# apple/ml-cvnets

Hardware: NVIDIA H100
Metric: images/sec training step, MobileViTv2-1.0 bf16 256x256 (higher is better)
Workload: dtype bf16

## Files before the change

### ml-cvnets_b200/csrc/common.cuh

```cuda
#pragma once
#include <cuda_bf16.h>
#include <cuda_runtime.h>
#include <stdint.h>
#include <stdio.h>
#include <string.h>

#include "../../include/cvnets_b200.h"

#if defined(__CUDA_ARCH__) && (__CUDA_ARCH__ != 900)
#error "libcvnets_b200 targets sm_90a (H100) only"
#endif

typedef __nv_bfloat16 bf16;
typedef __nv_bfloat162 bf162;

void cvb_set_error(const char* fmt, ...);
#define CVB_CHECK(cond, ...)            \
  do {                                  \
    if (!(cond)) {                      \
      cvb_set_error(__VA_ARGS__);       \
      return 1;                         \
    }                                   \
  } while (0)
#define CVB_CUDA(call)                                                                   \
  do {                                                                                   \
    cudaError_t e_ = (call);                                                             \
    if (e_ != cudaSuccess) {                                                             \
      (void)cudaGetLastError();  \
      cvb_set_error("%s:%d CUDA error: %s", __FILE__, __LINE__, cudaGetErrorString(e_)); \
      return 2;                                                                          \
    }                                                                                    \
  } while (0)
#define CVB_LAUNCH_CHECK() CVB_CUDA(cudaGetLastError())

static inline bool cvb_aligned16(const void* p) { return (reinterpret_cast<uintptr_t>(p) & 15) == 0; }
int cvb_num_sms();
int cvb_det_alloc(double** scratch, size_t n, cudaStream_t st);
int cvb_det_add(const double* scratch, float* dst, int rows, int cols, int ld, cudaStream_t st);
int cvb_det_free(double* scratch, cudaStream_t st);

#ifndef CVB_SILU_EXP
#define CVB_SILU_EXP 0
#endif
__device__ __forceinline__ float tanh_approx_f(float x) {
  float y;
  asm("tanh.approx.f32 %0, %1;" : "=f"(y) : "f"(x));
  return y;
}
__device__ __forceinline__ float sigmoid_f(float z) {
#if CVB_SILU_EXP
  return 1.0f / (1.0f + __expf(-z));
#else
  return fmaf(0.5f, tanh_approx_f(0.5f * z), 0.5f);
#endif
}
__device__ __forceinline__ float silu_f(float z) {
#if CVB_SILU_EXP
  return z / (1.0f + __expf(-z));
#else
  const float h = 0.5f * z;
  return fmaf(h, tanh_approx_f(h), h);
#endif
}
__device__ __forceinline__ float silu_grad_f(float z) {
  const float s = sigmoid_f(z);
  return s * (1.0f + z * (1.0f - s));
}
__device__ __forceinline__ float bf16_round(float x) { return __bfloat162float(__float2bfloat16_rn(x)); }

__device__ __forceinline__ uint32_t pack_bf162(float lo, float hi) {
  bf162 v = __floats2bfloat162_rn(lo, hi);
  return *reinterpret_cast<uint32_t*>(&v);
}
__device__ __forceinline__ float2 unpack_bf162(uint32_t u) {
  bf162 v = *reinterpret_cast<bf162*>(&u);
  return __bfloat1622float2(v);
}
__device__ __forceinline__ float2 ffma2(float2 a, float2 b, float2 c) { return make_float2(__fmaf_rn(a.x, b.x, c.x), __fmaf_rn(a.y, b.y, c.y)); }
__device__ __forceinline__ float2 fmul2(float2 a, float2 b) { return make_float2(__fmul_rn(a.x, b.x), __fmul_rn(a.y, b.y)); }
__device__ __forceinline__ float2 fadd2(float2 a, float2 b) { return make_float2(__fadd_rn(a.x, b.x), __fadd_rn(a.y, b.y)); }
__device__ __forceinline__ void unpack8(const uint4& u, float* f) {
  float2 a = unpack_bf162(u.x), b = unpack_bf162(u.y), c = unpack_bf162(u.z), d = unpack_bf162(u.w);
  f[0] = a.x; f[1] = a.y; f[2] = b.x; f[3] = b.y; f[4] = c.x; f[5] = c.y; f[6] = d.x; f[7] = d.y;
}
__device__ __forceinline__ uint4 pack8(const float* f) {
  uint4 u;
  u.x = pack_bf162(f[0], f[1]); u.y = pack_bf162(f[2], f[3]); u.z = pack_bf162(f[4], f[5]); u.w = pack_bf162(f[6], f[7]);
  return u;
}
__device__ __forceinline__ uint4 ldg16(const void* p) { return __ldg(reinterpret_cast<const uint4*>(p)); }
__device__ __forceinline__ uint4 ldg16_stream(const void* p) {
  uint4 r;
  asm volatile("ld.global.nc.L1::no_allocate.v4.u32 {%0,%1,%2,%3}, [%4];" : "=r"(r.x), "=r"(r.y), "=r"(r.z), "=r"(r.w) : "l"(p));
  return r;
}
__device__ __forceinline__ void stg16(void* p, const uint4& v) { *reinterpret_cast<uint4*>(p) = v; }

__device__ __forceinline__ uint32_t smem_u32(const void* p) { return static_cast<uint32_t>(__cvta_generic_to_shared(p)); }

__device__ __forceinline__ void cp_async16(uint32_t smem_addr, const void* gptr, bool pred) {
  int sz = pred ? 16 : 0;
  asm volatile("cp.async.cg.shared.global [%0], [%1], 16, %2;\n" ::"r"(smem_addr), "l"(gptr), "r"(sz));
}
__device__ __forceinline__ void cp_async_commit() { asm volatile("cp.async.commit_group;\n" ::); }
template <int N>
__device__ __forceinline__ void cp_async_wait() { asm volatile("cp.async.wait_group %0;\n" ::"n"(N)); }

__device__ __forceinline__ void ldmatrix_x4(uint32_t addr, uint32_t& r0, uint32_t& r1, uint32_t& r2, uint32_t& r3) {
  asm volatile("ldmatrix.sync.aligned.m8n8.x4.shared.b16 {%0,%1,%2,%3}, [%4];\n" : "=r"(r0), "=r"(r1), "=r"(r2), "=r"(r3) : "r"(addr));
}
__device__ __forceinline__ void ldmatrix_x4_trans(uint32_t addr, uint32_t& r0, uint32_t& r1, uint32_t& r2, uint32_t& r3) {
  asm volatile("ldmatrix.sync.aligned.m8n8.x4.trans.shared.b16 {%0,%1,%2,%3}, [%4];\n" : "=r"(r0), "=r"(r1), "=r"(r2), "=r"(r3) : "r"(addr));
}
__device__ __forceinline__ void mma_bf16_16816(float* d, const uint32_t* a, uint32_t b0, uint32_t b1) {
  asm volatile(
      "mma.sync.aligned.m16n8k16.row.col.f32.bf16.bf16.f32 {%0,%1,%2,%3}, {%4,%5,%6,%7}, {%8,%9}, {%0,%1,%2,%3};\n"
      : "+f"(d[0]), "+f"(d[1]), "+f"(d[2]), "+f"(d[3])
      : "r"(a[0]), "r"(a[1]), "r"(a[2]), "r"(a[3]), "r"(b0), "r"(b1));
}

__device__ __forceinline__ float warp_sum(float v) {
#pragma unroll
  for (int o = 16; o > 0; o >>= 1) v += __shfl_xor_sync(0xffffffffu, v, o);
  return v;
}
__device__ __forceinline__ float warp_max(float v) {
#pragma unroll
  for (int o = 16; o > 0; o >>= 1) v = fmaxf(v, __shfl_xor_sync(0xffffffffu, v, o));
  return v;
}

__device__ __forceinline__ float apply_mode(int mode, float x, float p0, float p1) {
  switch (mode) {
    case CVB_A_AFF: return fmaf(p0, x, p1);
    case CVB_A_AFF_SILU: return silu_f(fmaf(p0, x, p1));
    case CVB_A_SILU: return silu_f(x);
    default: return x;
  }
}

__device__ __forceinline__ void pdl_wait() { asm volatile("griddepcontrol.wait;" ::: "memory"); }
__device__ __forceinline__ void pdl_trigger() { asm volatile("griddepcontrol.launch_dependents;" ::: "memory"); }
int cvb_pdl_enabled();
template <typename... KArgs, typename... Args>
static inline cudaError_t cvb_launch(void (*kernel)(KArgs...), dim3 grid, dim3 block, size_t smem, cudaStream_t st, Args&&... args) {
  cudaLaunchConfig_t cfg;
  memset(&cfg, 0, sizeof(cfg));
  cfg.gridDim = grid;
  cfg.blockDim = block;
  cfg.dynamicSmemBytes = smem;
  cfg.stream = st;
  cudaLaunchAttribute attr[1];
  attr[0].id = cudaLaunchAttributeProgrammaticStreamSerialization;
  attr[0].val.programmaticStreamSerializationAllowed = 1;
  cfg.attrs = attr;
  cfg.numAttrs = cvb_pdl_enabled() ? 1 : 0;
  return cudaLaunchKernelEx(&cfg, kernel, static_cast<KArgs>(args)...);
}

#include <cuda.h>

int cvb_make_tmap_nhwc(CUtensorMap* map, const void* base, int B, int H, int W, int C, int boxH, int boxW, int boxC, int swizzle128);
int cvb_make_tmap_2d_k32(CUtensorMap* map, const void* base, int64_t rows, int cols, int ld, int box_rows);
int cvb_make_tmap_2d_c64(CUtensorMap* map, const void* base, int64_t rows, int cols, int ld, int box_rows);

__device__ __forceinline__ void mbar_init(uint64_t* bar, uint32_t count) {
  asm volatile("mbarrier.init.shared::cta.b64 [%0], %1;" ::"r"(smem_u32(bar)), "r"(count) : "memory");
}
__device__ __forceinline__ void fence_mbar_init() { asm volatile("fence.mbarrier_init.release.cluster;" ::: "memory"); }
__device__ __forceinline__ void fence_proxy_async() { asm volatile("fence.proxy.async.shared::cta;" ::: "memory"); }
__device__ __forceinline__ void mbar_expect_tx(uint64_t* bar, uint32_t bytes) {
  asm volatile("mbarrier.arrive.expect_tx.shared::cta.b64 _, [%0], %1;" ::"r"(smem_u32(bar)), "r"(bytes) : "memory");
}
__device__ __forceinline__ void mbar_wait(uint64_t* bar, uint32_t parity) {
  asm volatile(
      "{\n\t"
      ".reg .pred P1;\n\t"
      "WAIT_LOOP:\n\t"
      "mbarrier.try_wait.parity.shared::cta.b64 P1, [%0], %1;\n\t"
      "@P1 bra WAIT_DONE;\n\t"
      "bra WAIT_LOOP;\n\t"
      "WAIT_DONE:\n\t"
      "}" ::"r"(smem_u32(bar)), "r"(parity)
      : "memory");
}
__device__ __forceinline__ void tma_load_2d(void* smem_dst, const CUtensorMap* map, uint64_t* bar, int col, int row) {
  asm volatile("cp.async.bulk.tensor.2d.shared::cluster.global.mbarrier::complete_tx::bytes [%0], [%1, {%3, %4}], [%2];" ::"r"(smem_u32(smem_dst)),
               "l"(reinterpret_cast<uint64_t>(map)), "r"(smem_u32(bar)), "r"(col), "r"(row)
               : "memory");
}
__device__ __forceinline__ void mbar_arrive(uint64_t* bar) { asm volatile("mbarrier.arrive.shared::cta.b64 _, [%0];" ::"r"(smem_u32(bar)) : "memory"); }

enum { WG_SW128 = 1, WG_SW64 = 2 };
__device__ __forceinline__ uint64_t wgmma_desc(uint32_t saddr, uint32_t lbo_bytes, uint32_t sbo_bytes, int layout) {
  uint64_t d = 0;
  d |= (uint64_t)((saddr & 0x3FFFFu) >> 4);
  d |= (uint64_t)((lbo_bytes >> 4) & 0x3FFFu) << 16;
  d |= (uint64_t)((sbo_bytes >> 4) & 0x3FFFu) << 32;
  d |= (uint64_t)layout << 62;
  return d;
}
__device__ __forceinline__ void wgmma_fence() { asm volatile("wgmma.fence.sync.aligned;" ::: "memory"); }
__device__ __forceinline__ void wgmma_commit() { asm volatile("wgmma.commit_group.sync.aligned;" ::: "memory"); }
template <int N>
__device__ __forceinline__ void wgmma_wait() { asm volatile("wgmma.wait_group.sync.aligned %0;" ::"n"(N) : "memory"); }
template <int R>
__device__ __forceinline__ void wgmma_reg_fence(float* d) {
#pragma unroll
  for (int i = 0; i < R; ++i) asm volatile("" : "+f"(d[i])::"memory");
}

#define CVB_WG_R8(b) "+f"(d[b + 0]), "+f"(d[b + 1]), "+f"(d[b + 2]), "+f"(d[b + 3]), "+f"(d[b + 4]), "+f"(d[b + 5]), "+f"(d[b + 6]), "+f"(d[b + 7])
template <int TA, int TB>
__device__ __forceinline__ void wgmma_m64n64(float* d, uint64_t da, uint64_t db, uint32_t accumulate) {
  asm volatile(
      "{\n\t.reg .pred p;\n\tsetp.ne.b32 p, %34, 0;\n\t"
      "wgmma.mma_async.sync.aligned.m64n64k16.f32.bf16.bf16 "
      "{%0,%1,%2,%3,%4,%5,%6,%7,%8,%9,%10,%11,%12,%13,%14,%15,%16,%17,%18,%19,%20,%21,%22,%23,%24,%25,%26,%27,%28,%29,%30,%31}, "
      "%32, %33, p, 1, 1, %35, %36;\n\t}"
      : CVB_WG_R8(0), CVB_WG_R8(8), CVB_WG_R8(16), CVB_WG_R8(24)
      : "l"(da), "l"(db), "r"(accumulate), "n"(TA), "n"(TB));
}
template <int TA, int TB>
__device__ __forceinline__ void wgmma_m64n128(float* d, uint64_t da, uint64_t db, uint32_t accumulate) {
  asm volatile(
      "{\n\t.reg .pred p;\n\tsetp.ne.b32 p, %66, 0;\n\t"
      "wgmma.mma_async.sync.aligned.m64n128k16.f32.bf16.bf16 "
      "{%0,%1,%2,%3,%4,%5,%6,%7,%8,%9,%10,%11,%12,%13,%14,%15,%16,%17,%18,%19,%20,%21,%22,%23,%24,%25,%26,%27,%28,%29,%30,%31,"
      "%32,%33,%34,%35,%36,%37,%38,%39,%40,%41,%42,%43,%44,%45,%46,%47,%48,%49,%50,%51,%52,%53,%54,%55,%56,%57,%58,%59,%60,%61,%62,%63}, "
      "%64, %65, p, 1, 1, %67, %68;\n\t}"
      : CVB_WG_R8(0), CVB_WG_R8(8), CVB_WG_R8(16), CVB_WG_R8(24), CVB_WG_R8(32), CVB_WG_R8(40), CVB_WG_R8(48), CVB_WG_R8(56)
      : "l"(da), "l"(db), "r"(accumulate), "n"(TA), "n"(TB));
}
template <int TB>
__device__ __forceinline__ void wgmma_m64n64_rs(float* d, const uint32_t* a, uint64_t db, uint32_t accumulate) {
  asm volatile(
      "{\n\t.reg .pred p;\n\tsetp.ne.b32 p, %37, 0;\n\t"
      "wgmma.mma_async.sync.aligned.m64n64k16.f32.bf16.bf16 "
      "{%0,%1,%2,%3,%4,%5,%6,%7,%8,%9,%10,%11,%12,%13,%14,%15,%16,%17,%18,%19,%20,%21,%22,%23,%24,%25,%26,%27,%28,%29,%30,%31}, "
      "{%32,%33,%34,%35}, %36, p, 1, 1, %38;\n\t}"
      : CVB_WG_R8(0), CVB_WG_R8(8), CVB_WG_R8(16), CVB_WG_R8(24)
      : "r"(a[0]), "r"(a[1]), "r"(a[2]), "r"(a[3]), "l"(db), "r"(accumulate), "n"(TB));
}
#undef CVB_WG_R8

__device__ __forceinline__ void tma_load_4d(void* smem_dst, const CUtensorMap* map, uint64_t* bar, int c, int w, int h, int b) {
  asm volatile("cp.async.bulk.tensor.4d.shared::cluster.global.mbarrier::complete_tx::bytes [%0], [%1, {%3, %4, %5, %6}], [%2];" ::"r"(
                   smem_u32(smem_dst)),
               "l"(reinterpret_cast<uint64_t>(map)), "r"(smem_u32(bar)), "r"(c), "r"(w), "r"(h), "r"(b)
               : "memory");
}
```

### ml-cvnets_b200/csrc/gemm_tc.cu

```cuda
#include "common.cuh"
#include <cstdlib>

namespace {

constexpr int TC_BM = 128;
constexpr int TC_BN = 128;
constexpr int TC_BK = 32;
constexpr int TC_STAGE = TC_BM * TC_BK * 2;
constexpr int TC_WBLK = TC_BN * TC_BK * 2;
constexpr int TC_LDO = TC_BN + 8;
constexpr int TC_EPI_THREADS = 256;
constexpr int TC_PRODUCER_WARP = TC_EPI_THREADS / 32;
constexpr int TC_THREADS = TC_EPI_THREADS + 32;
constexpr int TC_XF_THREADS_MAX = 256;
template <int AMODE>
struct XfCfg {
  static constexpr int THREADS = (AMODE == CVB_A_RAW) ? 0 : (AMODE == CVB_A_BNB ? 128 : TC_XF_THREADS_MAX);
  static constexpr int IT = THREADS ? (TC_BM * 4) / THREADS : 1;
};
constexpr int TC_MAX_STAGES = 12;

enum { TEPI_STORE = 0, TEPI_STORE_R = 1, TEPI_SILU_BWD = 2, TEPI_GN_BWD = 3 };

__device__ __forceinline__ uint64_t desc_sw64(uint32_t saddr) { return wgmma_desc(saddr, 16, 512, WG_SW64); }
__device__ __forceinline__ void epi_bar_sync() { asm volatile("bar.sync 1, %0;" ::"n"(TC_EPI_THREADS) : "memory"); }

template <int AMODE, int EPI, bool WRES>
__global__ void __launch_bounds__(TC_THREADS + XfCfg<AMODE>::THREADS, 1)
    pw_gemm_tc_kernel(const __grid_constant__ CUtensorMap tmA, const __grid_constant__ CUtensorMap tmA2, const __grid_constant__ CUtensorMap tmW,
                      const cvb_gemm_args p, int NST) {
  constexpr bool XF = (AMODE != CVB_A_RAW);
  constexpr bool TWO_A = (AMODE == CVB_A_BNB);
  constexpr bool HAS_P = (AMODE == CVB_A_AFF || AMODE == CVB_A_AFF_SILU || AMODE == CVB_A_GN || AMODE == CVB_A_BNB);
  const int tid = threadIdx.x, lane = tid & 31, warp = tid >> 5;
  const int n0 = blockIdx.x * TC_BN;
  const int KT = (p.K + TC_BK - 1) / TC_BK;
  const int m_tiles = (p.M + TC_BM - 1) / TC_BM;
  const int my_tiles = (m_tiles - (int)blockIdx.y + (int)gridDim.y - 1) / (int)gridDim.y;
  const int total = my_tiles * KT;

  extern __shared__ __align__(1024) uint8_t smem_raw[];
  uint8_t* smem = smem_raw + ((1024u - (smem_u32(smem_raw) & 1023u)) & 1023u);
  constexpr int A_BYTES = (TWO_A ? 2 : 1) * TC_STAGE;
  constexpr int RING_STAGE = A_BYTES + (WRES ? 0 : TC_WBLK);
  uint8_t* sW = smem;
  uint8_t* sA = sW + (WRES ? KT * TC_WBLK : 0);
  uint8_t* sO = sA + NST * RING_STAGE;
  float* sP = reinterpret_cast<float*>(sO + TC_BM * TC_LDO * 2);
  __shared__ __align__(8) uint64_t full[TC_MAX_STAGES], empty[TC_MAX_STAGES], ready[TC_MAX_STAGES];
  __shared__ __align__(8) uint64_t wbar;
  __shared__ double s_samp[2][128];

  if (tid == 0) {
    for (int i = 0; i < NST; ++i) { mbar_init(&full[i], 1); mbar_init(&empty[i], 2); mbar_init(&ready[i], XfCfg<AMODE>::THREADS ? XfCfg<AMODE>::THREADS / 32 : 1); }
    mbar_init(&wbar, 1);
    fence_mbar_init();
  }
  if (tid < 128) { s_samp[0][tid] = 0.0; s_samp[1][tid] = 0.0; }
  __syncthreads();
  pdl_wait();
  pdl_trigger();

  if (warp == TC_PRODUCER_WARP) {
    if (lane == 0) {
      if (WRES) {
        mbar_expect_tx(&wbar, (uint32_t)KT * TC_WBLK);
        for (int kt = 0; kt < KT; ++kt) tma_load_2d(sW + kt * TC_WBLK, &tmW, &wbar, kt * TC_BK, n0);
      }
      for (int it = 0; it < total; ++it) {
        const int stage = it % NST;
        if (it >= NST) mbar_wait(&empty[stage], ((it / NST) - 1) & 1);
        const int j = it / KT, kt = it - j * KT;
        const int m0 = ((int)blockIdx.y + j * (int)gridDim.y) * TC_BM;
        mbar_expect_tx(&full[stage], RING_STAGE);
        tma_load_2d(sA + stage * RING_STAGE, &tmA, &full[stage], kt * TC_BK, m0);
        if (TWO_A) tma_load_2d(sA + stage * RING_STAGE + TC_STAGE, &tmA2, &full[stage], kt * TC_BK, m0);
        if (!WRES) tma_load_2d(sA + stage * RING_STAGE + A_BYTES, &tmW, &full[stage], kt * TC_BK, n0);
      }
    }
  } else if (warp > TC_PRODUCER_WARP) {
    if (XF) {
      constexpr int TC_XF_THREADS = XfCfg<AMODE>::THREADS > 0 ? XfCfg<AMODE>::THREADS : 128;
      constexpr int TC_XF_IT = XfCfg<AMODE>::IT;
      const int tt = tid - TC_THREADS;
      const int Kpad = KT * TC_BK;
      if (HAS_P) {
        for (int k = tt; k < Kpad; k += TC_XF_THREADS) {
          const bool ok = k < p.K;
          sP[k] = ok ? p.a_p0[k] : 0.f;
          sP[Kpad + k] = ok ? p.a_p1[k] : 0.f;
          if (AMODE == CVB_A_BNB) sP[2 * Kpad + k] = ok ? p.a_p2[k] : 0.f;
        }
        asm volatile("bar.sync 2, %0;" ::"n"(TC_XF_THREADS) : "memory");
      }
      float tmu[TC_XF_IT], trs[TC_XF_IT];
#pragma unroll
      for (int i = 0; i < TC_XF_IT; ++i) { tmu[i] = 0.f; trs[i] = 1.f; }
      for (int it = 0; it < total; ++it) {
        const int stage = it % NST;
        const int j = it / KT, kt = it - j * KT;
        const int m0 = ((int)blockIdx.y + j * (int)gridDim.y) * TC_BM;
        const int k0 = kt * TC_BK;
        if (AMODE == CVB_A_GN && kt == 0) {
#pragma unroll
          for (int i = 0; i < TC_XF_IT; ++i) {
            const int m = m0 + (tt >> 2) + i * (TC_XF_THREADS / 4);
            const int b = (m < p.M ? m : p.M - 1) / p.rows_per_sample;
            tmu[i] = __ldg(p.row_mean + b);
            trs[i] = __ldg(p.row_rstd + b);
          }
        }
        mbar_wait(&full[stage], (it / NST) & 1);
        uint8_t* st = sA + stage * RING_STAGE;
#pragma unroll
        for (int i = 0; i < TC_XF_IT; ++i) {
          const int c = tt + i * TC_XF_THREADS;
          const int row = c >> 2, ch = c & 3;
          const int k = k0 + ch * 8;
          const uint32_t off = (uint32_t)(row * 64 + ((ch ^ ((row >> 1) & 3)) << 4));
          uint4* pa = reinterpret_cast<uint4*>(st + off);
          float f[8], q0[8], q1[8];
          unpack8(*pa, f);
          if (HAS_P) {
            *reinterpret_cast<float4*>(q0) = *reinterpret_cast<const float4*>(sP + k);
            *reinterpret_cast<float4*>(q0 + 4) = *reinterpret_cast<const float4*>(sP + k + 4);
            *reinterpret_cast<float4*>(q1) = *reinterpret_cast<const float4*>(sP + Kpad + k);
            *reinterpret_cast<float4*>(q1 + 4) = *reinterpret_cast<const float4*>(sP + Kpad + k + 4);
          }
          if (AMODE == CVB_A_AFF) {
#pragma unroll
            for (int e = 0; e < 8; ++e) f[e] = fmaf(q0[e], f[e], q1[e]);
          } else if (AMODE == CVB_A_AFF_SILU) {
#pragma unroll
            for (int e = 0; e < 8; ++e) f[e] = silu_f(fmaf(q0[e], f[e], q1[e]));
          } else if (AMODE == CVB_A_SILU) {
#pragma unroll
            for (int e = 0; e < 8; ++e) f[e] = silu_f(f[e]);
          } else if (AMODE == CVB_A_GN) {
#pragma unroll
            for (int e = 0; e < 8; ++e) f[e] = fmaf((f[e] - tmu[i]) * trs[i], q0[e], q1[e]);
          } else if (AMODE == CVB_A_BNB) {
            float y[8], q2[8];
            unpack8(*reinterpret_cast<const uint4*>(st + TC_STAGE + off), y);
            *reinterpret_cast<float4*>(q2) = *reinterpret_cast<const float4*>(sP + 2 * Kpad + k);
            *reinterpret_cast<float4*>(q2 + 4) = *reinterpret_cast<const float4*>(sP + 2 * Kpad + k + 4);
#pragma unroll
            for (int e = 0; e < 8; ++e) f[e] = fmaf(q0[e], f[e], fmaf(q1[e], y[e], q2[e]));
          }
          *pa = (m0 + row < p.M) ? pack8(f) : make_uint4(0u, 0u, 0u, 0u);
        }
        fence_proxy_async();
        __syncwarp();
        if (lane == 0) mbar_arrive(&ready[stage]);
      }
    }
  } else {
    const int et = tid;
    const int wg = tid >> 7;
    const int r0 = wg * 64 + ((tid & 127) >> 5) * 16 + (lane >> 2);
    const int pc = 2 * (lane & 3);
    int chn[2];
    bool ch_ok[2];
    float bias[2], ep0[2], ep1[2];
#pragma unroll
    for (int h = 0; h < 2; ++h) {
      chn[h] = n0 + r0 + 8 * h;
      ch_ok[h] = chn[h] < p.N;
      bias[h] = (ch_ok[h] && p.bias) ? __ldg(p.bias + chn[h]) : 0.f;
      ep0[h] = ((EPI == TEPI_SILU_BWD || EPI == TEPI_GN_BWD) && ch_ok[h] && p.e_p0) ? __ldg(p.e_p0 + chn[h]) : 1.f;
      ep1[h] = (EPI == TEPI_SILU_BWD && ch_ok[h] && p.e_p1) ? __ldg(p.e_p1 + chn[h]) : 0.f;
    }
    constexpr bool has_aux = (EPI != TEPI_STORE);
    const bf16* __restrict__ AUX = static_cast<const bf16*>(EPI == TEPI_STORE_R ? p.R : p.Y);
    const int ldaux = EPI == TEPI_STORE_R ? p.ldr : p.ldy;
    const bool want_samp = (p.samp_sum != nullptr) && (EPI != TEPI_GN_BWD);
    const bool lin_bwd = (p.e_mode == CVB_E_LIN_BWD);
    const int rps = p.rows_per_sample > 0 ? p.rows_per_sample : 1;
    float cs[2] = {0.f, 0.f}, cq[2] = {0.f, 0.f};
    bf16* __restrict__ Cg = static_cast<bf16*>(p.C);
    constexpr int CGS = TC_BN / 8;
    const uint32_t w_off = (uint32_t)wg * 64 * 64;

    auto issue_aux = [&](int j) {
      const int m0 = ((int)blockIdx.y + j * (int)gridDim.y) * TC_BM;
      for (int c = et; c < TC_BM * CGS; c += TC_EPI_THREADS) {
        const int row = c / CGS, cgc = c % CGS;
        const int m = m0 + row, n = n0 + cgc * 8;
        const bool ok = (m < p.M) && (n < p.N);
        cp_async16(smem_u32(sO + row * (TC_LDO * 2) + cgc * 16), AUX + (ok ? (size_t)m * ldaux + n : 0), ok);
      }
      cp_async_commit();
    };
    if (has_aux && my_tiles > 0) issue_aux(0);
    if (WRES) mbar_wait(&wbar, 0);

    float acc[64];
    int it = 0;
    for (int j = 0; j < my_tiles; ++j) {
      const int m0 = ((int)blockIdx.y + j * (int)gridDim.y) * TC_BM;
      for (int kt = 0; kt < KT; ++kt, ++it) {
        const int stage = it % NST;
        mbar_wait(XF ? &ready[stage] : &full[stage], (it / NST) & 1);
        const uint32_t aa = smem_u32(sA + stage * RING_STAGE);
        const uint32_t wa = (WRES ? smem_u32(sW + kt * TC_WBLK) : aa + A_BYTES) + w_off;
        wgmma_fence();
#pragma unroll
        for (int k = 0; k < TC_BK / 16; ++k) wgmma_m64n128<0, 0>(acc, desc_sw64(wa + k * 32), desc_sw64(aa + k * 32), (kt | k) ? 1u : 0u);
        wgmma_commit();
        wgmma_wait<1>();
        if (kt > 0 && (tid & 127) == 0) mbar_arrive(&empty[(it - 1) % NST]);
      }
      wgmma_wait<0>();
      wgmma_reg_fence<64>(acc);
      if ((tid & 127) == 0) mbar_arrive(&empty[(it - 1) % NST]);

      if (has_aux) {
        cp_async_wait<0>();
        epi_bar_sync();
      }
      const bool full_tile = (m0 + TC_BM <= p.M);
      float gs[2][2] = {{0.f, 0.f}, {0.f, 0.f}}, gq[2][2] = {{0.f, 0.f}, {0.f, 0.f}};
#pragma unroll
      for (int h = 0; h < 2; ++h) {
        bf16* so = reinterpret_cast<bf16*>(sO) + r0 + 8 * h;
        if (full_tile && !has_aux) {
#pragma unroll
          for (int jb = 0; jb < 16; ++jb) {
#pragma unroll
            for (int e = 0; e < 2; ++e) {
              const float v = acc[4 * jb + 2 * h + e] + bias[h];
              so[(8 * jb + pc + e) * TC_LDO] = __float2bfloat16_rn(v);
              cs[h] += v;
              cq[h] = fmaf(v, v, cq[h]);
            }
          }
        } else {
#pragma unroll
          for (int jb = 0; jb < 16; ++jb) {
#pragma unroll
            for (int e = 0; e < 2; ++e) {
              const int i = 8 * jb + pc + e;
              float v = acc[4 * jb + 2 * h + e] + ((full_tile || m0 + i < p.M) ? bias[h] : 0.f);
              float y = 0.f;
              if (has_aux) y = __bfloat162float(so[i * TC_LDO]);
              if (EPI == TEPI_STORE_R) v += y;
              if (EPI == TEPI_SILU_BWD && !lin_bwd) v *= silu_grad_f(fmaf(ep0[h], y, ep1[h]));
              if (EPI == TEPI_GN_BWD) {
                gs[h][jb >> 3] += v;
                gq[h][jb >> 3] = fmaf(v, y, gq[h][jb >> 3]);
                so[i * TC_LDO] = __float2bfloat16_rn(v * ep0[h]);
              } else {
                const bf16 vb = __float2bfloat16_rn(v);
                so[i * TC_LDO] = vb;
                const float vr = __bfloat162float(vb);
                cs[h] += vr;
                cq[h] = fmaf(vr, EPI == TEPI_SILU_BWD ? y : vr, cq[h]);
              }
            }
          }
        }
      }
      if (EPI == TEPI_GN_BWD) {
        const int nsamples = (p.M + rps - 1) / rps;
#pragma unroll
        for (int h = 0; h < 2; ++h) {
#pragma unroll
          for (int hf = 0; hf < 2; ++hf) {
            float a = gs[h][hf], bx = gq[h][hf];
            a += __shfl_xor_sync(0xffffffffu, a, 1);
            a += __shfl_xor_sync(0xffffffffu, a, 2);
            bx += __shfl_xor_sync(0xffffffffu, bx, 1);
            bx += __shfl_xor_sync(0xffffffffu, bx, 2);
            const int mh = m0 + hf * 64;
            if ((lane & 3) == 0 && ch_ok[h] && mh < p.M) {
              double* wsA = p.gn_ws + (size_t)(mh / rps) * p.N + chn[h];
              atomicAdd(wsA, (double)a);
              atomicAdd(wsA + (size_t)nsamples * p.N, (double)bx);
            }
          }
        }
      }
      epi_bar_sync();
      const int first_sample = m0 / rps;
      for (int c = et; c < TC_BM * CGS; c += TC_EPI_THREADS) {
        const int row = c / CGS, cgc = c % CGS;
        const int m = m0 + row, n = n0 + cgc * 8;
        const uint4 u = *reinterpret_cast<const uint4*>(sO + row * (TC_LDO * 2) + cgc * 16);
        if (m < p.M && n < p.N) stg16(Cg + (size_t)m * p.ldc + n, u);
        if (want_samp) {
          float f[8];
          unpack8(u, f);
          float sv = 0.f, sq = 0.f;
#pragma unroll
          for (int e = 0; e < 8; ++e) { sv += f[e]; sq = fmaf(f[e], f[e], sq); }
#pragma unroll
          for (int o = CGS / 2; o > 0; o >>= 1) {
            sv += __shfl_xor_sync(0xffffffffu, sv, o);
            sq += __shfl_xor_sync(0xffffffffu, sq, o);
          }
          if (cgc == 0 && m < p.M) {
            atomicAdd(&s_samp[0][m / rps - first_sample], (double)sv);
            atomicAdd(&s_samp[1][m / rps - first_sample], (double)sq);
          }
        }
      }
      epi_bar_sync();
      if (want_samp) {
        const int mlast = min(m0 + TC_BM, p.M) - 1;
        const int nsamp = mlast / rps - first_sample + 1;
        if (et < nsamp) {
          atomicAdd(p.samp_sum + first_sample + et, s_samp[0][et]);
          atomicAdd(p.samp_sq + first_sample + et, s_samp[1][et]);
          s_samp[0][et] = 0.0;
          s_samp[1][et] = 0.0;
        }
      }
      if (has_aux && j + 1 < my_tiles) issue_aux(j + 1);
    }
    if (EPI != TEPI_GN_BWD) {
#pragma unroll
      for (int h = 0; h < 2; ++h) {
        float s = cs[h], q = cq[h];
        s += __shfl_xor_sync(0xffffffffu, s, 1);
        s += __shfl_xor_sync(0xffffffffu, s, 2);
        q += __shfl_xor_sync(0xffffffffu, q, 1);
        q += __shfl_xor_sync(0xffffffffu, q, 2);
        if (p.col_sum && ch_ok[h] && (lane & 3) == 0) {
          atomicAdd(p.col_sum + chn[h], (double)s);
          atomicAdd(p.col_sq + chn[h], (double)q);
        }
      }
    }
  }
}

template <int AMODE, int EPI, bool WRES>
int launch_tc_impl(const cvb_gemm_args& a, cudaStream_t st, size_t fixed, int stage_bytes) {
  const size_t budget = (size_t)216 * 1024;
  int nst = (int)((budget - fixed) / stage_bytes);
  if (nst > TC_MAX_STAGES) nst = TC_MAX_STAGES;
  const size_t smem = fixed + (size_t)nst * stage_bytes;
  static bool attr = false;
  if (!attr) {
    CVB_CUDA(cudaFuncSetAttribute(pw_gemm_tc_kernel<AMODE, EPI, WRES>, cudaFuncAttributeMaxDynamicSharedMemorySize, 216 * 1024));
    attr = true;
  }
  const int n_tiles = (a.N + TC_BN - 1) / TC_BN, m_tiles = (a.M + TC_BM - 1) / TC_BM;
  int gy = cvb_num_sms() / n_tiles;
  if (gy > m_tiles) gy = m_tiles;
  if (gy < 1) gy = 1;
  CUtensorMap tmA, tmA2, tmW;
  if (cvb_make_tmap_2d_k32(&tmA, a.A, a.M, a.K, a.lda, TC_BM)) return 1;
  if (cvb_make_tmap_2d_k32(&tmA2, AMODE == CVB_A_BNB ? a.A2 : a.A, a.M, a.K, AMODE == CVB_A_BNB ? a.lda2 : a.lda, TC_BM)) return 1;
  if (cvb_make_tmap_2d_k32(&tmW, a.W, a.N, a.K, a.ldw, TC_BN)) return 1;
  dim3 grid(n_tiles, gy);
  const int threads = TC_THREADS + XfCfg<AMODE>::THREADS;
  CVB_CUDA(cvb_launch(pw_gemm_tc_kernel<AMODE, EPI, WRES>, grid, threads, smem, st, tmA, tmA2, tmW, a, nst));
  CVB_LAUNCH_CHECK();
  return 0;
}

template <int AMODE, int EPI>
int launch_tc(const cvb_gemm_args& a, cudaStream_t st) {
  const int KT = (a.K + TC_BK - 1) / TC_BK;
  const int nvec = (AMODE == CVB_A_AFF || AMODE == CVB_A_AFF_SILU || AMODE == CVB_A_GN) ? 2 : (AMODE == CVB_A_BNB ? 3 : 0);
  const int a_bytes = (AMODE == CVB_A_BNB ? 2 : 1) * TC_STAGE;
  const size_t stagebuf = (size_t)TC_BM * TC_LDO * 2 + (size_t)nvec * KT * TC_BK * 4 + 1024;
  const size_t panel = (size_t)KT * TC_WBLK;
  if (panel + stagebuf + 6 * (size_t)a_bytes <= (size_t)216 * 1024) return launch_tc_impl<AMODE, EPI, true>(a, st, panel + stagebuf, a_bytes);
  return launch_tc_impl<AMODE, EPI, false>(a, st, stagebuf, a_bytes + TC_WBLK);
}

__global__ void __launch_bounds__(128) gn_bwd_ws_finalize_kernel(const double* __restrict__ ws, const float* __restrict__ mean,
                                                                  const float* __restrict__ rstd, const float* __restrict__ gamma, int B, int N,
                                                                  double* col_sum, double* col_sq, double* samp_sum, double* samp_sq) {
  pdl_wait();
  pdl_trigger();
  __shared__ double s_red[2][4];
  const int b = blockIdx.x, tid = threadIdx.x;
  if (b >= B) {
    __shared__ double s_col[2][8][16];
    const int cl = tid & 15, sg = tid >> 4, c = (b - B) * 16 + cl;
    double sa = 0.0, st = 0.0;
    if (c < N) {
#pragma unroll 4
      for (int s = sg; s < B; s += 8) {
        const double A = ws[(size_t)s * N + c], Bx = ws[((size_t)B + s) * N + c];
        sa += A;
        st += (double)rstd[s] * (Bx - (double)mean[s] * A);
      }
    }
    s_col[0][sg][cl] = sa;
    s_col[1][sg][cl] = st;
    __syncthreads();
    if (sg == 0 && c < N) {
      for (int g = 1; g < 8; ++g) { sa += s_col[0][g][cl]; st += s_col[1][g][cl]; }
      col_sum[c] += sa;
      col_sq[c] += st;
    }
    return;
  }
  const double mu = (double)mean[b], rs = (double)rstd[b];
  double sg = 0.0, sgx = 0.0;
  for (int c = tid; c < N; c += 128) {
    const double A = ws[(size_t)b * N + c], Bx = ws[((size_t)B + b) * N + c];
    const double t = rs * (Bx - mu * A);
    const double gm = gamma ? (double)gamma[c] : 1.0;
    sg += gm * A;
    sgx += gm * t;
  }
#pragma unroll
  for (int o = 16; o > 0; o >>= 1) {
    sg += __shfl_xor_sync(0xffffffffu, sg, o);
    sgx += __shfl_xor_sync(0xffffffffu, sgx, o);
  }
  if ((tid & 31) == 0) { s_red[0][tid >> 5] = sg; s_red[1][tid >> 5] = sgx; }
  __syncthreads();
  if (tid == 0 && samp_sum) {
    atomicAdd(samp_sum + b, s_red[0][0] + s_red[0][1] + s_red[0][2] + s_red[0][3]);
    atomicAdd(samp_sq + b, s_red[1][0] + s_red[1][1] + s_red[1][2] + s_red[1][3]);
  }
}

template <int AMODE>
int launch_tc_gn_bwd(const cvb_gemm_args& a, cudaStream_t st) {
  int rc = launch_tc<AMODE, TEPI_GN_BWD>(a, st);
  if (rc != 0) return rc;
  const int B = (a.M + a.rows_per_sample - 1) / a.rows_per_sample;
  const int col_blocks = a.col_sum ? (a.N + 15) / 16 : 0;
  CVB_CUDA(cvb_launch(gn_bwd_ws_finalize_kernel, B + col_blocks, 128, 0, st, static_cast<const double*>(a.gn_ws), a.row_mean, a.row_rstd, a.e_p0, B, a.N, a.col_sum,
                      a.col_sq, a.samp_sum, a.samp_sq));
  CVB_LAUNCH_CHECK();
  return 0;
}

template <int AMODE>
int dispatch_tc_epi(const cvb_gemm_args& a, cudaStream_t st) {
  if (a.e_mode == CVB_E_GN_BWD && a.gn_ws && a.rows_per_sample % (TC_BM / 2) == 0 && !a.bias && (AMODE == CVB_A_RAW || AMODE == CVB_A_BNB))
    return launch_tc_gn_bwd<AMODE == CVB_A_BNB ? CVB_A_BNB : CVB_A_RAW>(a, st);
  if (a.e_mode == CVB_E_STORE) return a.R ? launch_tc<AMODE, TEPI_STORE_R>(a, st) : launch_tc<AMODE, TEPI_STORE>(a, st);
  if ((a.e_mode == CVB_E_SILU_BWD || a.e_mode == CVB_E_LIN_BWD) && (AMODE == CVB_A_RAW || AMODE == CVB_A_BNB)) return launch_tc<AMODE == CVB_A_BNB ? CVB_A_BNB : CVB_A_RAW, TEPI_SILU_BWD>(a, st);
  return -1;
}

}

int cvb_pw_gemm_tc(const cvb_gemm_args& a, cudaStream_t st) {
  static const int min_n = [] { const char* e = getenv("CVB_TC_MIN_N"); return e ? atoi(e) : 96; }();
  if (a.N < min_n || (a.N >= 96 && a.N % 128 != 0 && a.N % 128 < 64 && a.N < 256)) return -1;
  switch (a.a_mode) {
    case CVB_A_RAW: return dispatch_tc_epi<CVB_A_RAW>(a, st);
    case CVB_A_AFF: return dispatch_tc_epi<CVB_A_AFF>(a, st);
    case CVB_A_AFF_SILU: return dispatch_tc_epi<CVB_A_AFF_SILU>(a, st);
    case CVB_A_SILU: return dispatch_tc_epi<CVB_A_SILU>(a, st);
    case CVB_A_GN: return dispatch_tc_epi<CVB_A_GN>(a, st);
    case CVB_A_BNB: return dispatch_tc_epi<CVB_A_BNB>(a, st);
    default: return -1;
  }
}
```

Measured before the change: 6888.

## Use TMA for GEMM epilogue stores and aux tile loads with double-buffered staging

The pointwise GEMM epilogue now writes output tiles into a 128B-swizzled shared buffer and stores them with TMA bulk tensor stores, instead of per-thread 16-byte global stores. Auxiliary inputs (residual or Y) are loaded by the producer warp via TMA into double-buffered staging, synchronised with full/free mbarriers, replacing cp.async issued by the epilogue threads. This is meant to overlap output writeback and aux prefetch with the next tile's MMA and to free epilogue threads from address work. The cost is extra shared memory for the doubled output buffers, which can reduce pipeline stages, plus new synchronisation complexity.

```diff
diff --git a/ml-cvnets_b200/csrc/common.cuh b/ml-cvnets_b200/csrc/common.cuh
--- a/ml-cvnets_b200/csrc/common.cuh
+++ b/ml-cvnets_b200/csrc/common.cuh
@@ -190,6 +190,16 @@
                : "memory");
 }
 __device__ __forceinline__ void mbar_arrive(uint64_t* bar) { asm volatile("mbarrier.arrive.shared::cta.b64 _, [%0];" ::"r"(smem_u32(bar)) : "memory"); }
+__device__ __forceinline__ void tma_store_2d(const CUtensorMap* map, const void* smem_src, int col, int row) {
+  asm volatile("cp.async.bulk.tensor.2d.global.shared::cta.bulk_group [%0, {%2, %3}], [%1];" ::"l"(reinterpret_cast<uint64_t>(map)),
+               "r"(smem_u32(smem_src)), "r"(col), "r"(row)
+               : "memory");
+}
+__device__ __forceinline__ void bulk_commit() { asm volatile("cp.async.bulk.commit_group;" ::: "memory"); }
+template <int N>
+__device__ __forceinline__ void bulk_wait_read() { asm volatile("cp.async.bulk.wait_group.read %0;" ::"n"(N) : "memory"); }
+template <int N>
+__device__ __forceinline__ void bulk_wait() { asm volatile("cp.async.bulk.wait_group %0;" ::"n"(N) : "memory"); }
 
 enum { WG_SW128 = 1, WG_SW64 = 2 };
 __device__ __forceinline__ uint64_t wgmma_desc(uint32_t saddr, uint32_t lbo_bytes, uint32_t sbo_bytes, int layout) {
diff --git a/ml-cvnets_b200/csrc/gemm_tc.cu b/ml-cvnets_b200/csrc/gemm_tc.cu
--- a/ml-cvnets_b200/csrc/gemm_tc.cu
+++ b/ml-cvnets_b200/csrc/gemm_tc.cu
@@ -8,7 +8,8 @@
 constexpr int TC_BK = 32;
 constexpr int TC_STAGE = TC_BM * TC_BK * 2;
 constexpr int TC_WBLK = TC_BN * TC_BK * 2;
-constexpr int TC_LDO = TC_BN + 8;
+constexpr int TC_OHALF = TC_BM * 64 * 2;
+constexpr int TC_OBUF = 2 * TC_OHALF;
 constexpr int TC_EPI_THREADS = 256;
 constexpr int TC_PRODUCER_WARP = TC_EPI_THREADS / 32;
 constexpr int TC_THREADS = TC_EPI_THREADS + 32;
@@ -21,6 +22,8 @@
 constexpr int TC_MAX_STAGES = 12;
 
 enum { TEPI_STORE = 0, TEPI_STORE_R = 1, TEPI_SILU_BWD = 2, TEPI_GN_BWD = 3 };
+template <int EPI>
+constexpr int tc_obufs() { return EPI == TEPI_STORE ? 1 : 2; }
 
 __device__ __forceinline__ uint64_t desc_sw64(uint32_t saddr) { return wgmma_desc(saddr, 16, 512, WG_SW64); }
 __device__ __forceinline__ void epi_bar_sync() { asm volatile("bar.sync 1, %0;" ::"n"(TC_EPI_THREADS) : "memory"); }
@@ -28,8 +31,10 @@
 template <int AMODE, int EPI, bool WRES>
 __global__ void __launch_bounds__(TC_THREADS + XfCfg<AMODE>::THREADS, 1)
     pw_gemm_tc_kernel(const __grid_constant__ CUtensorMap tmA, const __grid_constant__ CUtensorMap tmA2, const __grid_constant__ CUtensorMap tmW,
-                      const cvb_gemm_args p, int NST) {
+                      const __grid_constant__ CUtensorMap tmX, const __grid_constant__ CUtensorMap tmC, const cvb_gemm_args p, int NST) {
   constexpr bool XF = (AMODE != CVB_A_RAW);
+  constexpr bool has_aux = (EPI != TEPI_STORE);
+  constexpr int NOB = tc_obufs<EPI>();
   constexpr bool TWO_A = (AMODE == CVB_A_BNB);
   constexpr bool HAS_P = (AMODE == CVB_A_AFF || AMODE == CVB_A_AFF_SILU || AMODE == CVB_A_GN || AMODE == CVB_A_BNB);
   const int tid = threadIdx.x, lane = tid & 31, warp = tid >> 5;
@@ -46,17 +51,23 @@
   uint8_t* sW = smem;
   uint8_t* sA = sW + (WRES ? KT * TC_WBLK : 0);
   uint8_t* sO = sA + NST * RING_STAGE;
-  float* sP = reinterpret_cast<float*>(sO + TC_BM * TC_LDO * 2);
+  float* sP = reinterpret_cast<float*>(sO + NOB * TC_OBUF);
   __shared__ __align__(8) uint64_t full[TC_MAX_STAGES], empty[TC_MAX_STAGES], ready[TC_MAX_STAGES];
   __shared__ __align__(8) uint64_t wbar;
+  __shared__ __align__(8) uint64_t xfull[2], xfree[2];
   __shared__ double s_samp[2][128];
 
   if (tid == 0) {
     for (int i = 0; i < NST; ++i) { mbar_init(&full[i], 1); mbar_init(&empty[i], 2); mbar_init(&ready[i], XfCfg<AMODE>::THREADS ? XfCfg<AMODE>::THREADS / 32 : 1); }
     mbar_init(&wbar, 1);
+    for (int b = 0; b < 2; ++b) { mbar_init(&xfull[b], 1); mbar_init(&xfree[b], 1); }
     fence_mbar_init();
   }
   if (tid < 128) { s_samp[0][tid] = 0.0; s_samp[1][tid] = 0.0; }
+  if (has_aux && n0 + 64 >= p.N) {
+    for (int i = tid; i < NOB * TC_OHALF / 16; i += (int)blockDim.x)
+      reinterpret_cast<uint4*>(sO + (i / (TC_OHALF / 16)) * TC_OBUF + TC_OHALF)[i % (TC_OHALF / 16)] = make_uint4(0u, 0u, 0u, 0u);
+  }
   __syncthreads();
   pdl_wait();
   pdl_trigger();
@@ -72,6 +83,13 @@
         if (it >= NST) mbar_wait(&empty[stage], ((it / NST) - 1) & 1);
         const int j = it / KT, kt = it - j * KT;
         const int m0 = ((int)blockIdx.y + j * (int)gridDim.y) * TC_BM;
+        if (has_aux && kt == 0) {
+          const int b = j & 1;
+          if (j >= 2) mbar_wait(&xfree[b], ((j >> 1) - 1) & 1);
+          const int halves = (n0 + 64 < p.N) ? 2 : 1;
+          mbar_expect_tx(&xfull[b], (uint32_t)halves * TC_OHALF);
+          for (int h = 0; h < halves; ++h) tma_load_2d(sO + b * TC_OBUF + h * TC_OHALF, &tmX, &xfull[b], n0 + 64 * h, m0);
+        }
         mbar_expect_tx(&full[stage], RING_STAGE);
         tma_load_2d(sA + stage * RING_STAGE, &tmA, &full[stage], kt * TC_BK, m0);
         if (TWO_A) tma_load_2d(sA + stage * RING_STAGE + TC_STAGE, &tmA2, &full[stage], kt * TC_BK, m0);
@@ -170,28 +188,12 @@
       ep0[h] = ((EPI == TEPI_SILU_BWD || EPI == TEPI_GN_BWD) && ch_ok[h] && p.e_p0) ? __ldg(p.e_p0 + chn[h]) : 1.f;
       ep1[h] = (EPI == TEPI_SILU_BWD && ch_ok[h] && p.e_p1) ? __ldg(p.e_p1 + chn[h]) : 0.f;
     }
-    constexpr bool has_aux = (EPI != TEPI_STORE);
-    const bf16* __restrict__ AUX = static_cast<const bf16*>(EPI == TEPI_STORE_R ? p.R : p.Y);
-    const int ldaux = EPI == TEPI_STORE_R ? p.ldr : p.ldy;
     const bool want_samp = (p.samp_sum != nullptr) && (EPI != TEPI_GN_BWD);
     const bool lin_bwd = (p.e_mode == CVB_E_LIN_BWD);
     const int rps = p.rows_per_sample > 0 ? p.rows_per_sample : 1;
     float cs[2] = {0.f, 0.f}, cq[2] = {0.f, 0.f};
-    bf16* __restrict__ Cg = static_cast<bf16*>(p.C);
     constexpr int CGS = TC_BN / 8;
     const uint32_t w_off = (uint32_t)wg * 64 * 64;
-
-    auto issue_aux = [&](int j) {
-      const int m0 = ((int)blockIdx.y + j * (int)gridDim.y) * TC_BM;
-      for (int c = et; c < TC_BM * CGS; c += TC_EPI_THREADS) {
-        const int row = c / CGS, cgc = c % CGS;
-        const int m = m0 + row, n = n0 + cgc * 8;
-        const bool ok = (m < p.M) && (n < p.N);
-        cp_async16(smem_u32(sO + row * (TC_LDO * 2) + cgc * 16), AUX + (ok ? (size_t)m * ldaux + n : 0), ok);
-      }
-      cp_async_commit();
-    };
-    if (has_aux && my_tiles > 0) issue_aux(0);
     if (WRES) mbar_wait(&wbar, 0);
 
     float acc[64];
@@ -207,6 +209,10 @@
 #pragma unroll
         for (int k = 0; k < TC_BK / 16; ++k) wgmma_m64n128<0, 0>(acc, desc_sw64(wa + k * 32), desc_sw64(aa + k * 32), (kt | k) ? 1u : 0u);
         wgmma_commit();
+        if (kt == 0 && tid == 0 && j > 0) {
+          bulk_wait_read<0>();
+          mbar_arrive(&xfree[(j - 1) % NOB]);
+        }
         wgmma_wait<1>();
         if (kt > 0 && (tid & 127) == 0) mbar_arrive(&empty[(it - 1) % NST]);
       }
@@ -214,22 +220,23 @@
       wgmma_reg_fence<64>(acc);
       if ((tid & 127) == 0) mbar_arrive(&empty[(it - 1) % NST]);
 
-      if (has_aux) {
-        cp_async_wait<0>();
-        epi_bar_sync();
-      }
+      uint8_t* const sOb = sO + (j % NOB) * TC_OBUF;
+      if (has_aux) mbar_wait(&xfull[j & 1], (j >> 1) & 1);
+      else if (j >= NOB) mbar_wait(&xfree[j % NOB], (j / NOB - 1) & 1);
       const bool full_tile = (m0 + TC_BM <= p.M);
       float gs[2][2] = {{0.f, 0.f}, {0.f, 0.f}}, gq[2][2] = {{0.f, 0.f}, {0.f, 0.f}};
 #pragma unroll
       for (int h = 0; h < 2; ++h) {
-        bf16* so = reinterpret_cast<bf16*>(sO) + r0 + 8 * h;
+        const int cl = (r0 & 63) + 8 * h;
+        uint8_t* const so_h = sOb + wg * TC_OHALF + (cl & 7) * 2;
+        auto so = [&](int jb, int e) { return reinterpret_cast<bf16*>(so_h + (8 * jb + pc + e) * 128 + (((cl >> 3) ^ (pc + e)) << 4)); };
         if (full_tile && !has_aux) {
 #pragma unroll
           for (int jb = 0; jb < 16; ++jb) {
 #pragma unroll
             for (int e = 0; e < 2; ++e) {
               const float v = acc[4 * jb + 2 * h + e] + bias[h];
-              so[(8 * jb + pc + e) * TC_LDO] = __float2bfloat16_rn(v);
+              *so(jb, e) = __float2bfloat16_rn(v);
               cs[h] += v;
               cq[h] = fmaf(v, v, cq[h]);
             }
@@ -242,16 +249,16 @@
               const int i = 8 * jb + pc + e;
               float v = acc[4 * jb + 2 * h + e] + ((full_tile || m0 + i < p.M) ? bias[h] : 0.f);
               float y = 0.f;
-              if (has_aux) y = __bfloat162float(so[i * TC_LDO]);
+              if (has_aux) y = __bfloat162float(*so(jb, e));
               if (EPI == TEPI_STORE_R) v += y;
               if (EPI == TEPI_SILU_BWD && !lin_bwd) v *= silu_grad_f(fmaf(ep0[h], y, ep1[h]));
               if (EPI == TEPI_GN_BWD) {
                 gs[h][jb >> 3] += v;
                 gq[h][jb >> 3] = fmaf(v, y, gq[h][jb >> 3]);
-                so[i * TC_LDO] = __float2bfloat16_rn(v * ep0[h]);
+                *so(jb, e) = __float2bfloat16_rn(v * ep0[h]);
               } else {
                 const bf16 vb = __float2bfloat16_rn(v);
-                so[i * TC_LDO] = vb;
+                *so(jb, e) = vb;
                 const float vr = __bfloat162float(vb);
                 cs[h] += vr;
                 cq[h] = fmaf(vr, EPI == TEPI_SILU_BWD ? y : vr, cq[h]);
@@ -280,14 +287,18 @@
           }
         }
       }
+      fence_proxy_async();
       epi_bar_sync();
-      const int first_sample = m0 / rps;
-      for (int c = et; c < TC_BM * CGS; c += TC_EPI_THREADS) {
-        const int row = c / CGS, cgc = c % CGS;
-        const int m = m0 + row, n = n0 + cgc * 8;
-        const uint4 u = *reinterpret_cast<const uint4*>(sO + row * (TC_LDO * 2) + cgc * 16);
-        if (m < p.M && n < p.N) stg16(Cg + (size_t)m * p.ldc + n, u);
-        if (want_samp) {
+      if (tid == 0) {
+        for (int h = 0; h < 2 && n0 + 64 * h < p.N; ++h) tma_store_2d(&tmC, sOb + h * TC_OHALF, n0 + 64 * h, m0);
+        bulk_commit();
+      }
+      if (want_samp) {
+        const int first_sample = m0 / rps;
+        for (int c = et; c < TC_BM * CGS; c += TC_EPI_THREADS) {
+          const int row = c / CGS, cgc = c % CGS;
+          const int m = m0 + row;
+          const uint4 u = *reinterpret_cast<const uint4*>(sOb + (cgc >> 3) * TC_OHALF + row * 128 + (((cgc & 7) ^ (row & 7)) << 4));
           float f[8];
           unpack8(u, f);
           float sv = 0.f, sq = 0.f;
@@ -303,9 +314,7 @@
             atomicAdd(&s_samp[1][m / rps - first_sample], (double)sq);
           }
         }
-      }
-      epi_bar_sync();
-      if (want_samp) {
+        epi_bar_sync();
         const int mlast = min(m0 + TC_BM, p.M) - 1;
         const int nsamp = mlast / rps - first_sample + 1;
         if (et < nsamp) {
@@ -315,8 +324,8 @@
           s_samp[1][et] = 0.0;
         }
       }
-      if (has_aux && j + 1 < my_tiles) issue_aux(j + 1);
-    }
+    }
+    if (tid == 0) bulk_wait<0>();
     if (EPI != TEPI_GN_BWD) {
 #pragma unroll
       for (int h = 0; h < 2; ++h) {
@@ -349,13 +358,16 @@
   int gy = cvb_num_sms() / n_tiles;
   if (gy > m_tiles) gy = m_tiles;
   if (gy < 1) gy = 1;
-  CUtensorMap tmA, tmA2, tmW;
+  CUtensorMap tmA, tmA2, tmW, tmX, tmC;
   if (cvb_make_tmap_2d_k32(&tmA, a.A, a.M, a.K, a.lda, TC_BM)) return 1;
   if (cvb_make_tmap_2d_k32(&tmA2, AMODE == CVB_A_BNB ? a.A2 : a.A, a.M, a.K, AMODE == CVB_A_BNB ? a.lda2 : a.lda, TC_BM)) return 1;
   if (cvb_make_tmap_2d_k32(&tmW, a.W, a.N, a.K, a.ldw, TC_BN)) return 1;
+  if (cvb_make_tmap_2d_c64(&tmC, a.C, a.M, a.N, a.ldc, TC_BM)) return 1;
+  if (EPI == TEPI_STORE) tmX = tmC;
+  else if (cvb_make_tmap_2d_c64(&tmX, EPI == TEPI_STORE_R ? a.R : a.Y, a.M, a.N, EPI == TEPI_STORE_R ? a.ldr : a.ldy, TC_BM)) return 1;
   dim3 grid(n_tiles, gy);
   const int threads = TC_THREADS + XfCfg<AMODE>::THREADS;
-  CVB_CUDA(cvb_launch(pw_gemm_tc_kernel<AMODE, EPI, WRES>, grid, threads, smem, st, tmA, tmA2, tmW, a, nst));
+  CVB_CUDA(cvb_launch(pw_gemm_tc_kernel<AMODE, EPI, WRES>, grid, threads, smem, st, tmA, tmA2, tmW, tmX, tmC, a, nst));
   CVB_LAUNCH_CHECK();
   return 0;
 }
@@ -365,7 +377,7 @@
   const int KT = (a.K + TC_BK - 1) / TC_BK;
   const int nvec = (AMODE == CVB_A_AFF || AMODE == CVB_A_AFF_SILU || AMODE == CVB_A_GN) ? 2 : (AMODE == CVB_A_BNB ? 3 : 0);
   const int a_bytes = (AMODE == CVB_A_BNB ? 2 : 1) * TC_STAGE;
-  const size_t stagebuf = (size_t)TC_BM * TC_LDO * 2 + (size_t)nvec * KT * TC_BK * 4 + 1024;
+  const size_t stagebuf = (size_t)tc_obufs<EPI>() * TC_OBUF + (size_t)nvec * KT * TC_BK * 4 + 1024;
   const size_t panel = (size_t)KT * TC_WBLK;
   if (panel + stagebuf + 6 * (size_t)a_bytes <= (size_t)216 * 1024) return launch_tc_impl<AMODE, EPI, true>(a, st, panel + stagebuf, a_bytes);
   return launch_tc_impl<AMODE, EPI, false>(a, st, stagebuf, a_bytes + TC_WBLK);
```

After: 7030, median of 6. +2.1%, better.
